# simonamtoft/downsampled-diffusion

Measured on AMD Instinct MI355X. Metric: images/sec (T=1000 sampling), 256x256 dDDPM-x3, higher is better.
Workload: dtype f32

## Files before the change

### downsampled-diffusion_amd/csrc/conv_igemm.hip

```cpp
#include <cstdlib>

#include "conv_common.h"

namespace ddk {

struct IgemmParams {
    const float* src0;
    const float* src1;
    const float* w;
    const float* bias;
    const float* resid;
    float* out;
    int c0, c1, cin;
    int B, H, W;
    int Hm, Wm;
    int Ho, Wo;
    int N, M;
    int in_stride, out_scale;
    int ntaps, nphase;
    int splits, kiters, kiters_per_split;
    long long slab_stride;
    int pre_mish, post_mish;
    float* mish_out;
    const float* dmish_src;
// ... 1161 lines not shown
        san::extent("conv resid", a.resid, pix_out * a.N * 4);
        san::extent("conv bias", a.bias, (long long)a.N * 4);
        san::extent("conv workspace", a.workspace, (long long)a.workspace_bytes);
        san::extent("conv mish_out", a.mish_out, pix_out * a.N * 4);
        san::extent("conv dmish_src", a.dmish_src, pix_out * a.N * 4);
        if (a.gn_partials && a.gn_groups > 0) san::extent("conv gn_partials", a.gn_partials, (pix_out / 128) * a.gn_groups * 8);
    }
#endif
    DDK_REQUIRE(aligned16(a.mish_out) && aligned16(a.dmish_src), "conv: mish_out / dmish_src alignment");
    DDK_REQUIRE(!(a.mish_out || a.dmish_src) || !(a.defer_reduce || a.gn_partials || fuse || ln),
                "conv: mish_out / dmish_src go with a plain conv (no deferred reduce, GroupNorm partials or LayerNorm folding)");
    const bool act_epilogue = a.mish_out || a.dmish_src;
    if (a.weight_wino && !a.pre_mish && !act_epilogue && conv_wino_ok(a.kind, a.H, a.W, a.c0 + a.c1, a.N)) {
        DDK_REQUIRE(aligned16(a.weight_wino), "conv: weight_wino alignment");
        DDK_TRY(ensure_device_init());
        const int ws = conv_wino_splits(a.B, a.H, a.W, a.c0 + a.c1, a.N);
        const long long slab = (long long)a.B * a.H * a.W * a.N;
        if (ws > 1) {
            const size_t need = (size_t)(fuse ? ws - 1 : ws) * slab * sizeof(float);
            if (!a.workspace || a.workspace_bytes < need) {
                set_error("conv(wino): split-K workspace too small (%zu < %zu)", a.workspace_bytes, need);
                return DDK_ERR_WORKSPACE;
            }
            DDK_REQUIRE(aligned16(a.workspace), "conv: workspace alignment");
        }
        DDK_REQUIRE((long long)a.B * a.H * a.W * (a.c0 > a.c1 ? a.c0 : a.c1) * 4 < (1LL << 31), "conv(wino): a source of 2 GiB or more");
        DDK_TRY(conv_wino_forward(a, ws, st, fuse));
        if (ws > 1 && !a.defer_reduce && !fuse) {
            const long long n4 = slab / 4;
            const int blocks = (int)(ceil_div(n4, 256) < 2048 ? ceil_div(n4, 256) : 2048);
            hipLaunchKernelGGL(splitk_reduce_kernel, dim3(blocks), dim3(256), 0, st, static_cast<const float*>(a.workspace), ws, slab, a.bias,
// ... 160 lines not shown
```

### downsampled-diffusion_amd/csrc/conv_wino.hip

```cpp
#include <atomic>
#include <cstdlib>
#include <type_traits>
#include <utility>

#include "cluster_sync.h"
#include "conv_common.h"
#include "pack_elems.h"

namespace ddk {

__device__ __attribute__((aligned(128))) float g_wino_zero[32];

struct WinoParams {
    const float* src0;
    const float* src1;
    const float* wu;
    const float* bias;
    const float* resid;
    float* out;
    int c0, c1, cin;
    int B, H, W, TH, TW;
    int N, tiles;
    int splits, chunks, chunks_per_split;
    long long slab_stride;
// ... 551 lines not shown
    DDK_HIP(hipFuncSetAttribute(reinterpret_cast<const void*>(&convT_wino_kernel<1>), hipFuncAttributeMaxDynamicSharedMemorySize,
                                (int)(WT_LDS_FL * sizeof(float))));
#endif
    DDK_HIP(hipFuncSetAttribute(reinterpret_cast<const void*>(&conv3x3_wino_kernel<0>), hipFuncAttributeMaxDynamicSharedMemorySize,
                                (int)(W_LDS_FLOATS * sizeof(float))));
    DDK_HIP(hipFuncSetAttribute(reinterpret_cast<const void*>(&conv3x3_wino_kernel<0, true>), hipFuncAttributeMaxDynamicSharedMemorySize,
                                (int)(W_LDS_FLOATS * sizeof(float))));
    DDK_HIP(hipFuncSetAttribute(reinterpret_cast<const void*>(&conv3x3_wino2_kernel<2, 0, false>), hipFuncAttributeMaxDynamicSharedMemorySize,
                                (int)(W2<2>::LDS_FL * sizeof(float))));
    DDK_HIP(hipFuncSetAttribute(reinterpret_cast<const void*>(&conv3x3_wino2_kernel<2, 0, true>), hipFuncAttributeMaxDynamicSharedMemorySize,
                                (int)(W2<2>::LDS_FL * sizeof(float))));
    DDK_HIP(hipFuncSetAttribute(reinterpret_cast<const void*>(&conv3x3_wino2_kernel<4, 0, false>), hipFuncAttributeMaxDynamicSharedMemorySize,
                                (int)(W2<4>::LDS_FL * sizeof(float))));
    DDK_HIP(hipFuncSetAttribute(reinterpret_cast<const void*>(&conv3x3_wino2_kernel<4, 0, true>), hipFuncAttributeMaxDynamicSharedMemorySize,
                                (int)(W2<4>::LDS_FL * sizeof(float))));
#ifdef DDK_TUNING
#define W2_DBG_ATTR(P_, D_) DDK_HIP(hipFuncSetAttribute(reinterpret_cast<const void*>(&conv3x3_wino2_kernel<P_, D_, false>), \
                                                hipFuncAttributeMaxDynamicSharedMemorySize, (int)(W2<P_>::LDS_FL * sizeof(float))))
    W2_DBG_ATTR(2, 1); W2_DBG_ATTR(2, 7); W2_DBG_ATTR(2, 9); W2_DBG_ATTR(2, 15); W2_DBG_ATTR(2, 17);
    W2_DBG_ATTR(4, 1); W2_DBG_ATTR(4, 7); W2_DBG_ATTR(4, 9); W2_DBG_ATTR(4, 15); W2_DBG_ATTR(4, 17);
#undef W2_DBG_ATTR
    DDK_HIP(hipFuncSetAttribute(reinterpret_cast<const void*>(&conv3x3_wino_kernel<1>), hipFuncAttributeMaxDynamicSharedMemorySize, (int)(W_LDS_FLOATS * sizeof(float))));
    DDK_HIP(hipFuncSetAttribute(reinterpret_cast<const void*>(&conv3x3_wino_kernel<2>), hipFuncAttributeMaxDynamicSharedMemorySize, (int)(W_LDS_FLOATS * sizeof(float))));
    DDK_HIP(hipFuncSetAttribute(reinterpret_cast<const void*>(&conv3x3_wino_kernel<3>), hipFuncAttributeMaxDynamicSharedMemorySize, (int)(W_LDS_FLOATS * sizeof(float))));
    DDK_HIP(hipFuncSetAttribute(reinterpret_cast<const void*>(&conv3x3_wino_kernel<4>), hipFuncAttributeMaxDynamicSharedMemorySize, (int)(W_LDS_FLOATS * sizeof(float))));
#endif
    return DDK_OK;
}

int conv_wino_cluster_np(int B, int H, int W, int cin, int N, int groups) {
// ... 12 lines not shown
int conv_wino_cluster_split_np(int B, int H, int W, int cin, int N, int groups, int* splits_out) {
    if (!conv_wino_ok(DDK_CONV3X3_S1, H, W, cin, N)) return 0;
    const int splits = conv_wino_splits(B, H, W, cin, N);
    if (splits_out) *splits_out = splits;
    if (splits <= 1 || splits > 4) return 0;
    const int np = wino_stats_shape_parts(B, H, W, cin, N, groups);
    if (np <= 0 || np > 8) return 0;
    const int variant = wino_variant(B, H, W, N);
    if (variant != WINO_V_D) return 0;
    const int nt_w = wino_nt(variant);
    if (N / groups > 32 || nt_w % (N / groups) || nt_w / (N / groups) > 8) return 0;
    const long long mt = (long long)B * np, nt = N / nt_w;
    if (mt * nt * splits > 256) return 0;
    return np;
}
size_t conv_wino_cluster_pair_words(int B, int H, int W, int N) {
    return (size_t)ceil_div((long long)B * (H / 2) * (W / 2), WBT) * (size_t)(N / WBN) * 16;
}
size_t conv_wino_cluster_ws_floats(int B, int H, int W, int N) {
    const long long mt = (long long)B * (H / 2) * (W / 2) / WBT, nt = N / WBN;
    return (size_t)(mt * nt * 32 + (long long)B * nt * 16);
}

bool conv_wino_cluster_device_ok() {
    static std::atomic<int> cached[64];
    int dev = 0;
    if (hipGetDevice(&dev) != hipSuccess || dev < 0 || dev >= 64) return false;
    int v = cached[dev].load(std::memory_order_relaxed);
    if (v == 0) {
        int cus = 0, xccs = 0;
        bool ok = hipDeviceGetAttribute(&cus, hipDeviceAttributeMultiprocessorCount, dev) == hipSuccess && cus == 256;
        ok = ok && hipDeviceGetAttribute(&xccs, hipDeviceAttributeNumberOfXccs, dev) == hipSuccess && xccs == 8;
        ok = ok && !getenv("HSA_CU_MASK") && !getenv("ROC_GLOBAL_CU_MASK");
        (void)hipGetLastError();
        v = ok ? 1 : 2;
        cached[dev].store(v, std::memory_order_relaxed);
    }
    return v == 1;
}

bool conv_wino_variant_new(int B, int H, int W, int N) { return wino_variant(B, H, W, N) != WINO_V_OLD; }

int conv_wino_forward(const ddk_conv_args& a, int splits, hipStream_t st, const WinoGnFuse* fuse) {
    WinoParams p{};
    if (fuse) {
        const int np = splits == 1 ? conv_wino_cluster_np(a.B, a.H, a.W, a.c0 + a.c1, a.N, fuse->groups)
                                   : conv_wino_cluster_split_np(a.B, a.H, a.W, a.c0 + a.c1, a.N, fuse->groups, nullptr);
        DDK_REQUIRE(np > 0 && !a.post_mish && !a.gn_partials, "conv(wino): shape not eligible for the in-launch GroupNorm");
        if (splits > 1) {
            DDK_REQUIRE(fuse->pairs && a.workspace && aligned16(a.workspace) && !fuse->res_x,
                        "conv(wino, cluster): a split shape needs pair counters and the slab workspace");
            p.cl_slab = static_cast<float*>(a.workspace);
            p.cl_pair = fuse->pairs;
        }
        DDK_REQUIRE(fuse->gamma && fuse->beta && fuse->records && fuse->counters && aligned16(fuse->gamma) && aligned16(fuse->beta) &&
                        aligned16(fuse->temb) && fuse->temb_stride % 4 == 0 && aligned16(fuse->records) && aligned16(fuse->counters),
                    "conv(wino): in-launch GroupNorm arguments");
        p.gn_gamma = fuse->gamma; p.gn_beta = fuse->beta; p.gn_temb = fuse->temb; p.gn_temb_rows = fuse->temb_rows;
        p.gn_temb_stride = fuse->temb_stride; p.gn_eps = fuse->eps;
        p.cl_rec = fuse->records; p.cl_cnt = fuse->counters; p.cl_fail = fuse->fail; p.cl_np = np;
        if (fuse->res_x) {
            DDK_REQUIRE(fuse->res_w && fuse->res_cin > 0 && fuse->res_cin <= 8 && fuse->res_ld >= fuse->res_cin && !a.resid,
// ... 13 lines not shown
        p.cpg = a.N / a.gn_groups;
    }
    p.src0 = a.src0; p.src1 = a.src1; p.wu = a.weight_wino; p.bias = a.bias; p.resid = a.resid; p.out = a.out;
    p.c0 = a.c0; p.c1 = a.c1; p.cin = a.c0 + a.c1;
    p.B = a.B; p.H = a.H; p.W = a.W; p.TH = a.H / 2; p.TW = a.W / 2;
    p.N = a.N; p.tiles = a.B * p.TH * p.TW;
    p.chunks = p.cin / 32;
    p.chunks_per_split = (int)ceil_div(p.chunks, splits);
    p.splits = (int)ceil_div(p.chunks, p.chunks_per_split);
    p.slab_stride = (long long)a.B * a.H * a.W * a.N;
    p.post_mish = a.post_mish;
    p.dTW = make_fastdiv_u((unsigned)p.TW);
    p.dTH = make_fastdiv_u((unsigned)p.TH);
    if (p.splits > 1 && !fuse) p.out = static_cast<float*>(a.workspace);
    const int variant = wino_variant(a.B, a.H, a.W, a.N);
    if (variant != WINO_V_OLD) {
        dim3 grid2((unsigned)ceil_div(p.tiles, WBT), (unsigned)(a.N / wino_nt(variant)), (unsigned)p.splits);
        const bool f = variant == WINO_V_F;
        const size_t lds = (size_t)(f ? W2<2>::LDS_FL : W2<4>::LDS_FL) * sizeof(float);
#ifdef DDK_TUNING
        if (getenv("DDK_WINO_STAMPS")) {
            const int v = getenv("DDK_WINO_DEBUG") ? atoi(getenv("DDK_WINO_DEBUG")) : 1;
#define W2_DBG_LAUNCH(D_)                                                                                              \
    if (v == D_) {                                                                                                     \
        if (f) hipLaunchKernelGGL((conv3x3_wino2_kernel<2, D_, false>), grid2, dim3(768), lds, st, p);                 \
        else hipLaunchKernelGGL((conv3x3_wino2_kernel<4, D_, false>), grid2, dim3(768), lds, st, p);                   \
        return check_launch("conv3x3_wino2_kernel<dbg>");                                                              \
    }
            W2_DBG_LAUNCH(7) W2_DBG_LAUNCH(9) W2_DBG_LAUNCH(15) W2_DBG_LAUNCH(17)
#undef W2_DBG_LAUNCH
// ... 145 lines not shown
}

extern "C" int ddk_conv3x3_gn_mish_cluster(const float* src0, int c0, const float* src1, int c1, const float* weight_wino, const float* bias,
                                           const float* gamma, const float* beta, const float* temb, int temb_stride, const float* addend,
                                           float* out, int B, int H, int W, int N, int groups, float eps, void* workspace,
                                           size_t workspace_bytes, ddk_stream_t s) {
    using namespace ddk;
    DDK_REQUIRE(src0 && weight_wino && gamma && beta && out && workspace, "conv3x3_gn_mish_cluster: null pointer");
    DDK_REQUIRE(conv_wino_cluster_device_ok() && ddk_conv3x3_gn_mish_cluster_ok(B, H, W, c0 + c1, N, groups) > 0,
                "conv3x3_gn_mish_cluster: shape or device not eligible (ddk_conv3x3_gn_mish_cluster_ok)");
    const size_t plain_bytes = ddk_conv3x3_gn_mish_cluster_workspace_bytes(B, H, W, N);
    const size_t split_bytes = ddk_conv3x3_gn_mish_cluster_split_workspace_bytes(B, H, W, c0 + c1, N, groups);
    DDK_REQUIRE(workspace_bytes >= (split_bytes ? split_bytes : plain_bytes) && aligned16(workspace), "conv3x3_gn_mish_cluster: workspace");
    float* ws = static_cast<float*>(workspace);
    DDK_HIP(hipMemsetAsync(ws, 0, ((size_t)B * 8 * 16 + 16) * sizeof(float), as_stream(s)));
    float* pairs = ws + plain_bytes / sizeof(float);
    if (split_bytes) DDK_HIP(hipMemsetAsync(pairs, 0, conv_wino_cluster_pair_words(B, H, W, N) * sizeof(float), as_stream(s)));
    ddk_conv_args a{};
    a.kind = DDK_CONV3X3_S1;
    a.src0 = src0; a.src1 = src1; a.c0 = c0; a.c1 = c1;
    a.weight = weight_wino;
    a.weight_wino = weight_wino;
    a.bias = bias;
    a.resid = addend;
    a.out = out;
    a.B = B; a.H = H; a.W = W; a.N = N;
    const ClWords w = cl_words(ws, B);
    WinoGnFuse f{gamma, beta, temb, nullptr, temb_stride, eps, groups, ws + (size_t)B * 8 * 16 + 16, w.counters, w.fail};
    if (split_bytes) {
        f.pairs = reinterpret_cast<unsigned*>(pairs);
        a.workspace = pairs + conv_wino_cluster_pair_words(B, H, W, N);
        a.workspace_bytes = split_bytes - plain_bytes - conv_wino_cluster_pair_words(B, H, W, N) * sizeof(float);
    }
    return conv_forward(a, as_stream(s), nullptr, &f);
}
```

### downsampled-diffusion_amd/csrc/conv_wino2_kernel.inc

```

template <int... I, class F>
__device__ __forceinline__ void static_for_impl(std::integer_sequence<int, I...>, F&& f) { (f(std::integral_constant<int, I>{}), ...); }
template <int N, class F>
__device__ __forceinline__ void static_for(F&& f) { static_for_impl(std::make_integer_sequence<int, N>{}, f); }

#ifndef DDK_WINO2_LP_F
#define DDK_WINO2_LP_F 8
#endif
#ifndef DDK_WINO2_LP_D
#define DDK_WINO2_LP_D 4
#endif
template <int P>
struct W2 {
    static constexpr int NT = 256 / P;
    static constexpr int NB = NT / 32;
    static constexpr int SPC = 16 / P;
    static constexpr int SPR = 4 / P;
    static constexpr int V_FL = P * WBT * 32;
    static constexpr int U_FL = P * NT * 32;
    static constexpr int STAGE = V_FL + U_FL;
    static constexpr int PPI = NT / 8;
    static constexpr int TP = NT + 4;
    static constexpr int T_FL = 4 * 2 * WBT * TP;
    static constexpr int LDS_FL = (3 * STAGE > T_FL + 320) ? 3 * STAGE : T_FL + 320;
    static constexpr int QUADS = NT / 4;
    static constexpr int ITEMS = 2 * WBT * QUADS / 512;
    static constexpr int LPL = P == 2 ? DDK_WINO2_LP_F : DDK_WINO2_LP_D;
    static constexpr int LPM = (32 - 4 * LPL) / 8;
    static_assert(4 * LPL + 8 * LPM == 32 && LPL % 2 == 0 && LPM % 2 == 0, "piece split: (8,0), (4,2) or (0,4)");
};
#ifndef DDK_WINO2_STAGGER
#define DDK_WINO2_STAGGER 1
#endif
constexpr bool W2_STAGGER = DDK_WINO2_STAGGER != 0;

__device__ unsigned long long g_wino_timeline[12 * 8 * 2];

template <int P, int DBG, bool CL>
__global__ __launch_bounds__(768) void conv3x3_wino2_kernel(const WinoParams p) {
    using G = W2<P>;
    constexpr int NT = G::NT, SPC = G::SPC, SPR = G::SPR, STAGE = G::STAGE, V_FL = G::V_FL;
    extern __shared__ __attribute__((aligned(16))) float smem[];
    unsigned long long r_entry = 0;
    if (DBG) r_entry = __builtin_amdgcn_s_memrealtime();
    const int tid = threadIdx.x, lane = tid & 63;
    const int wid = __builtin_amdgcn_readfirstlane(tid >> 6);
    int tile_m, tile_n, split;
    {
        const int nwg = gridDim.x * gridDim.y * gridDim.z;
        const int bid = blockIdx.x + gridDim.x * (blockIdx.y + gridDim.y * blockIdx.z);
        const int q = nwg >> 3, r = nwg & 7, xcd = bid & 7, idx = bid >> 3;
        const int logical = (xcd < r ? xcd * (q + 1) : r * (q + 1) + (xcd - r) * q) + idx;
        tile_n = logical % gridDim.y;
        const int rest = logical / gridDim.y;
        tile_m = rest % gridDim.x;
// ... 154 lines not shown
                unsigned long long tlA = 0;
                const bool tl = (DBG & 16) && blockIdx.x + blockIdx.y + blockIdx.z == 0 && S >= 8 && S < 16;
                if (tl) asm volatile("s_memtime %0\n\ts_waitcnt lgkmcnt(0)" : "=s"(tlA)::"memory");
                __builtin_amdgcn_s_barrier();
                if (tl) {
                    unsigned long long tlB;
                    asm volatile("s_memtime %0\n\ts_waitcnt lgkmcnt(0)" : "=s"(tlB)::"memory");
                    if (lane == 0) { g_wino_timeline[(wid * 8 + (S - 8)) * 2] = tlA; g_wino_timeline[(wid * 8 + (S - 8)) * 2 + 1] = tlB; }
                }
                b0 = b0 == 2 ? 0 : b0 + 1;
            });
        }
        return;
    }

    const int pp = wid % P, nb = wid / P;
    f32x16 acc[SPC];
#pragma unroll
    for (int i = 0; i < SPC; ++i)
#pragma unroll
        for (int r = 0; r < 16; ++r) acc[i][r] = 0.f;
    {
        const int fsw = ((lane & 31) >> 1) & 7, fh = lane >> 5;
        int foff[4];
#pragma unroll
        for (int q = 0; q < 4; ++q) foff[q] = (lane & 31) * 32 + (((2 * q + fh) ^ fsw) << 2);
        const int a_img = pp * (WBT * 32), b_img = V_FL + (pp * NT + nb * 32) * 32;
        if (G::LPM > 0 && !(DBG & 4)) {
            issue_u(0, 0, 4 * G::LPL + wid * G::LPM, std::integral_constant<int, G::LPM>{});
            issue_u(1, 1, 4 * G::LPL + wid * G::LPM, std::integral_constant<int, G::LPM>{});
            wait_vmcnt<G::LPM>();
// ... 66 lines not shown
                    if (more && !(DBG & 4)) wait_vmcnt<G::LPM>(); else wait_vmcnt<0>();
                    unsigned long long tA = 0, tB = 0;
                    if (DBG) { asm volatile("s_memtime %0\n\ts_waitcnt lgkmcnt(0)" : "=s"(tA)::"memory"); }
                    __builtin_amdgcn_s_barrier();
                    if (DBG) { asm volatile("s_memtime %0\n\ts_waitcnt lgkmcnt(0)" : "=s"(tB)::"memory"); c_wait += tB - tA; if (c_mma == 0) c_mma = tA; }
                    if ((DBG & 16) && blockIdx.x + blockIdx.y + blockIdx.z == 0 && S >= 8 && S < 16 && lane == 0) {
                        g_wino_timeline[(wid * 8 + (S - 8)) * 2] = tA;
                        g_wino_timeline[(wid * 8 + (S - 8)) * 2 + 1] = tB;
                    }
                    buf = nbuf;
                    ++S;
                });
            }
            if (STG) mma4(acc[SPC - 1], a[0], b[0]);
        };
        if (W2_STAGGER && wid >= 4) mloop(std::true_type{}); else mloop(std::false_type{});
        if (DBG && lane == 0 && wid == 0) {
            const int wg = (blockIdx.x + gridDim.x * (blockIdx.y + gridDim.y * blockIdx.z)) & 1023;
            unsigned long long tE;
            asm volatile("s_memtime %0\n\ts_waitcnt lgkmcnt(0)" : "=s"(tE)::"memory");
            g_wino_stamps[wg * 8 + 0] = r_entry;
            g_wino_stamps[wg * 8 + 1] = r_loop0;
            g_wino_stamps[wg * 8 + 2] = __builtin_amdgcn_s_memrealtime();
            g_wino_stamps[wg * 8 + 3] = c_wait;
            g_wino_stamps[wg * 8 + 4] = tE - c_mma;
            g_wino_stamps[wg * 8 + 5] = (unsigned long long)n_stages;
        }
    }
    {
        constexpr int TP = G::TP;
#pragma unroll
        for (int r = 0; r < 16; ++r) {
            const int row = (r & 3) + 8 * (r >> 2) + 4 * (lane >> 5);
            const int col = nb * 32 + (lane & 31);
            if constexpr (P == 4) {
                float* Ts = smem + pp * (2 * WBT * TP);
                const float m0 = acc[0][r], m1 = acc[1][r], m2 = acc[2][r], m3 = acc[3][r];
                Ts[row * TP + col] = (m0 + m1) + m2;
                Ts[(WBT + row) * TP + col] = (m1 - m2) - m3;
            } else {
                const float l0 = acc[0][r], l1 = acc[2][r], l2 = acc[4][r], l3 = acc[6][r];
                const float h0 = acc[1][r], h1 = acc[3][r], h2 = acc[5][r], h3 = acc[7][r];
                const float tl0 = (l0 + l1) + l2, tl1 = (l1 - l2) - l3;
                const float th0 = (h0 + h1) + h2, th1 = (h1 - h2) - h3;
                float* B0 = smem + (pp * 2 + 0) * (2 * WBT * TP);
                float* B1 = smem + (pp * 2 + 1) * (2 * WBT * TP);
                if (pp == 0) {
                    B0[row * TP + col] = tl0 + th0;          B0[(WBT + row) * TP + col] = tl1 + th1;
                    B1[row * TP + col] = -th0;               B1[(WBT + row) * TP + col] = -th1;
                } else {
                    B0[row * TP + col] = tl0;                B0[(WBT + row) * TP + col] = tl1;
                    B1[row * TP + col] = tl0 - th0;          B1[(WBT + row) * TP + col] = tl1 - th1;
                }
            }
        }
    }
    __syncthreads();

    constexpr int TP = G::TP, QUADS = G::QUADS, ITEMS = G::ITEMS;
    constexpr bool CLS = CL && P == 4;
    const bool partner = CLS && split > 0;
    const bool direct = p.splits == 1 || (CLS && !partner);
    float* outp = p.splits == 1 ? p.out : CLS ? p.cl_slab + (long long)(split - 1) * p.slab_stride : p.out + (long long)split * p.slab_stride;
    float4 keep[ITEMS][2];
    long long oo[ITEMS];
    int opix[ITEMS];
    const int cq = tid & (QUADS - 1);
    const int gn = n0 + cq * 4;
#pragma unroll
    for (int it = 0; it < ITEMS; ++it) {
        const int item = tid + it * 512;
        const int t = item / (2 * QUADS), a = (item / QUADS) & 1;
        const int g = t0 + t;
        keep[it][0] = keep[it][1] = make_float4(0.f, 0.f, 0.f, 0.f);
        oo[it] = -1;
        opix[it] = 0;
        if (g >= p.tiles || gn >= p.N) continue;
        const float* tp = smem + (a * WBT + t) * TP + cq * 4;
        const float4 q0 = *reinterpret_cast<const float4*>(tp);
        const float4 q1 = *reinterpret_cast<const float4*>(tp + 1 * (2 * WBT * TP));
        const float4 q2 = *reinterpret_cast<const float4*>(tp + 2 * (2 * WBT * TP));
        const float4 q3 = *reinterpret_cast<const float4*>(tp + 3 * (2 * WBT * TP));
        float4 y0, y1;
        if constexpr (P == 4) {
            y0 = f4add(f4add(q0, q1), q2);
            y1 = f4sub(f4sub(q1, q2), q3);
        } else {
            y0 = f4add(q0, q2);
            y1 = f4add(q1, q3);
        }
        const unsigned tmp = fdiv_u((unsigned)g, p.dTW);
        const int tx = g - (int)tmp * p.TW;
        const unsigned bq = fdiv_u(tmp, p.dTH);
        const int ty = (int)tmp - (int)bq * p.TH;
        const long long o0 = ((((long long)bq * p.H + 2 * ty + a) * p.W) + 2 * tx) * p.N + gn;
        oo[it] = o0;
        opix[it] = ((int)bq * p.H + 2 * ty + a) * p.W + 2 * tx;
        if (direct) {
            if (p.bias) {
// ... 8 lines not shown
            if (p.post_mish) {
                y0 = make_float4(mish_f(y0.x), mish_f(y0.y), mish_f(y0.z), mish_f(y0.w));
                y1 = make_float4(mish_f(y1.x), mish_f(y1.y), mish_f(y1.z), mish_f(y1.w));
            }
        }
        if (!CL) {
            *reinterpret_cast<float4*>(outp + o0) = y0;
            *reinterpret_cast<float4*>(outp + o0 + p.N) = y1;
        } else if (CLS && partner) {
            st_sc1_f4(outp + o0, y0);
            st_sc1_f4(outp + o0 + p.N, y1);
        }
        keep[it][0] = y0;
        keep[it][1] = y1;
    }
    if (CLS && p.splits > 1) {
        unsigned* pair = p.cl_pair + ((long long)tile_m * gridDim.y + tile_n) * 16;
        if (partner) {
            asm volatile("s_waitcnt vmcnt(0)" ::: "memory");
            __syncthreads();
            if (tid == 0) __hip_atomic_fetch_add(pair, 1u, __ATOMIC_RELAXED, __HIP_MEMORY_SCOPE_AGENT);
            return;
        }
        int* pair_gave_up = reinterpret_cast<int*>(smem + G::T_FL + 258);
        if (tid == 0) {
            *pair_gave_up = 0;
            const unsigned want = (unsigned)p.splits - 1u;
            if (cl_wait_ge<2>(pair, want, p.cl_fail)) *pair_gave_up = 1;
            __hip_atomic_store(pair, 0u, __ATOMIC_RELAXED, __HIP_MEMORY_SCOPE_AGENT);
        }
        __syncthreads();
// ... 155 lines not shown
```

### downsampled-diffusion_amd/csrc/ddk_internal.h

```cpp
#pragma once
#include <hip/hip_runtime.h>

#include <cstdarg>
#include <cstdint>
#include <cstdio>

#include "ddk.h"

#ifdef DDK_HOST_SANITIZE
#include "host_sanitize.h"
#endif

namespace ddk {

void set_error(const char* fmt, ...);

inline int fail_arg(const char* what) {
    set_error("bad argument: %s", what);
    return DDK_ERR_ARG;
}

inline int check_launch(const char* what) {
    hipError_t e = hipGetLastError();
    if (e != hipSuccess) {
// ... 93 lines not shown
    const float* c2;
    float eps;
};
struct WinoGnFuse {
    const float* gamma;
    const float* beta;
    const float* temb;
    const long long* temb_rows;
    int temb_stride;
    float eps;
    int groups;
    float* records;
    unsigned* counters;
    unsigned* fail;
    unsigned* pairs = nullptr;
    const float* res_x = nullptr;
    const float* res_w = nullptr;
    const float* res_b = nullptr;
    int res_cin = 0, res_ld = 0;
};
bool conv_ln_fold_ok(int B, int H, int W, int cin, int N);
int conv_forward(const ddk_conv_args& a, hipStream_t st, const ConvLnFold* ln = nullptr, const WinoGnFuse* fuse = nullptr);
int conv_splits(int kind, int B, int H, int W, int cin, int N);
bool conv_wino_ok(int kind, int H, int W, int cin, int N);
int conv_wino_splits(int B, int H, int W, int cin, int N);
int conv_wino_forward(const ddk_conv_args& a, int splits, hipStream_t st, const WinoGnFuse* fuse = nullptr);
int conv_wino_cluster_np(int B, int H, int W, int cin, int N, int groups);
int conv_wino_cluster_split_np(int B, int H, int W, int cin, int N, int groups, int* splits_out);
size_t conv_wino_cluster_pair_words(int B, int H, int W, int N);
bool conv_wino_variant_new(int B, int H, int W, int N);
bool conv_wino_cluster_device_ok();
size_t conv_wino_cluster_ws_floats(int B, int H, int W, int N);
unsigned conv_wino_cluster_timeouts();
unsigned conv_first_cluster_timeouts();
unsigned level_chain_cluster_timeouts();
struct ClWords { unsigned* counters; unsigned* fail; };
inline ClWords cl_words(float* cl, int B) { return {reinterpret_cast<unsigned*>(cl), reinterpret_cast<unsigned*>(cl + (size_t)B * 8 * 16)}; }
int cluster_fail_check(unsigned* word, hipStream_t st, const char* who, const char* tail);
bool convT_wino_ok(int H, int W, int cin, int N);
int convT_wino_splits(int B, int H, int W, int cin, int N);
int convT_wino_forward(const ddk_conv_args& a, int splits, hipStream_t st);
int conv_wino_init_device();
int conv_wino_stats_parts(int B, int H, int W, int cin, int N, int groups);
bool conv_first_ok(int cin, int N, int H, int W, int groups);
// ... 114 lines not shown
```

### downsampled-diffusion_amd/csrc/unet_plan.hip

```cpp
#include <algorithm>
#include <mutex>
#include <string>
#include <vector>

#include "ddk_internal.h"
#include "level_chain.h"

namespace ddk {

constexpr int HEADS = 4;
constexpr int HIDDEN = HEADS * 32;
constexpr int GROUPS = 8;
constexpr float GN_EPS = 1e-5f, LN_EPS = 1e-5f;

static inline int pad32(int c) { return (c + 31) / 32 * 32; }

enum PackKind { PK_COPY = 0, PK_CONV = 1, PK_CONVT = 2, PK_LINEAR_T = 3, PK_WINO = 4, PK_LOCAL = 5, PK_WLOCAL = 6, PK_FIRST = 7, PK_CONVT_WINO = 8,
                PK_ROWS = 9 , PK_LOCAL1 = 10 ,
                PK_CONVT_LOCAL = 11  };

struct Slot {
    std::string name;
    long long numel;
    int kind;
// ... 68 lines not shown
struct ddk_unet {
    std::mutex mu;
    std::vector<SamplerGraph> graphs;
    unsigned long long use_clock = 0;
    unsigned long long pack_epoch = 0;
    struct {
        const void* ws = nullptr;
        int t_start = -1, B = 0, H = 0, W = 0;
        unsigned long long pack_epoch = 0;
        std::vector<int64_t> map;
    } table;
    ddk_unet_config cfg;
    int cluster_gn = 1;
    int cluster_limit = 1 << 30;
    int cluster_np_max = 8;
    bool cluster_split = true;
    bool attn_kvctx = true;
    bool fold_down_reduce = false;
    bool first_gn = true;
    int level_chain = 9;
    int level_chain_max_batch = 32;
    int attn_fold_min_hw = 256;
    bool attn_fold = true;
    bool generic = false;
    std::vector<int> dimp;
    std::vector<Slot> slots;
    size_t packed_floats = 0;
    int L = 0;
    std::vector<int> dims;
    int time_dim = 0, temb_total = 0;
    size_t freqs = 0, w1t = 0, b1 = 0, w2t = 0, b2 = 0, temb_wt = 0, temb_bias = 0;
// ... 331 lines not shown
        std::lock_guard<std::mutex> lock(u->mu);
        u->cluster_limit = value;
        return DDK_OK;
    }
    if (option == 4) {
        std::lock_guard<std::mutex> lock(u->mu);
        if (!u->graphs.empty()) DDK_HIP(hipDeviceSynchronize());
        drop_graphs(u);
        u->cluster_np_max = value;
        return DDK_OK;
    }
    if (option == 11) {
        std::lock_guard<std::mutex> lock(u->mu);
        if (!u->graphs.empty()) DDK_HIP(hipDeviceSynchronize());
        drop_graphs(u);
        u->cluster_split = value != 0;
        return DDK_OK;
    }
    return fail_arg("unet_set_option: unknown option");
}
extern "C" unsigned ddk_debug_cluster_timeouts(void) {
    unsigned sum = 0;
    for (unsigned v : {ddk::conv_wino_cluster_timeouts(), ddk::conv_first_cluster_timeouts(), ddk::level_chain_cluster_timeouts()}) {
        if (v == ~0u) return ~0u;
        sum += v;
    }
    return sum;
}
extern "C" int ddk_unet_num_slots(const ddk_unet* u) { return u ? (int)u->slots.size() : 0; }
extern "C" const char* ddk_unet_slot_name(const ddk_unet* u, int slot) {
    return (u && slot >= 0 && slot < (int)u->slots.size()) ? u->slots[slot].name.c_str() : nullptr;
// ... 97 lines not shown
    return convT_wino_ok(H, W, cin, N) && convT_wino_splits(B, H, W, cin, N) <= 2;
}
static bool use_wino(const ConvW& cw, int H, int W, int cin, int N) {
    return cw.has_wu && conv_wino_ok(DDK_CONV3X3_S1, H, W, cin, N);
}
static int conv3_splits(const ConvW& cw, int B, int H, int W, int cin, int N) {
    return use_wino(cw, H, W, cin, N) ? conv_wino_splits(B, H, W, cin, N) : conv_splits(DDK_CONV3X3_S1, B, H, W, cin, N);
}
static size_t conv3_ws_floats(const ConvW& cw, int B, int H, int W, int cin, int N) {
    if (!use_wino(cw, H, W, cin, N)) return conv_workspace_bytes(DDK_CONV3X3_S1, B, H, W, cin, N) / 4;
    const int s = conv_wino_splits(B, H, W, cin, N);
    return s > 1 ? (size_t)s * B * H * W * N : 0;
}

constexpr size_t CL_PAIR_WORDS = 128 * 16;
static size_t cl_counter_floats(int B) { return (size_t)B * 8 * 16 + 16 + (size_t)B * 64 + CL_PAIR_WORDS; }
static size_t cl_chain_offset(int B) { return (size_t)B * 8 * 16 + 16; }
static size_t cl_pair_offset(int B) { return (size_t)B * 8 * 16 + 16 + (size_t)B * 64; }
constexpr int CHAIN_BUFS = 18;
constexpr int CHAIN8_BUFS = 5;

static void res_sizes(const ResW& r, int B, int H, int W, Layout& ly) {
    const size_t M = (size_t)B * H * W;
    upd(ly.act, M * r.co);
    upd(ly.splitk, conv3_ws_floats(r.c1, B, H, W, r.ci_pad, r.co));
    upd(ly.splitk, conv3_ws_floats(r.c2, B, H, W, r.co, r.co));
    if (r.has_res) upd(ly.splitk, conv_workspace_bytes(DDK_CONV1X1, B, H, W, r.ci_pad, r.co) / 4);
    upd(ly.gn_ws, groupnorm_workspace_bytes(B, H * W, r.co, GROUPS) / 4);
    upd(ly.gn_ws, (size_t)2 * GROUPS * (M / 128 + 1));
    upd(ly.cl, cl_counter_floats(B) + conv_wino_cluster_ws_floats(B, H, W, r.co));
    if (H * W % 128 == 0 && H * W / 128 <= 8) upd(ly.cl, cl_counter_floats(B) + conv_first_gn_ws_floats(B, H, W));
}

static void attn_sizes(const AttnW& a, int B, int H, int W, Layout& ly) {
    const size_t M = (size_t)B * H * W;
    upd(ly.act, M * a.c);
    upd(ly.qkv, M * 3 * HIDDEN);
    upd(ly.o, M * HIDDEN);
    upd(ly.ctx, (size_t)B * HEADS * 32 * 32);
    upd(ly.splitk, linattn_context_workspace_bytes(B, H * W, HEADS) / 4);
    if (attn_kvctx_ok(B, H * W, a.c, HEADS)) upd(ly.splitk, attn_kvctx_workspace_bytes(B, H * W) / 4);
    upd(ly.splitk, conv_workspace_bytes(DDK_CONV1X1, B, H, W, a.c, 3 * HIDDEN) / 4);
    upd(ly.splitk, conv_workspace_bytes(DDK_CONV1X1, B, H, W, HIDDEN, a.c) / 4);
}

// ... 140 lines not shown
    }
    const int cl_np = c.allow_cluster && cw.has_wu && conv_wino_cluster_device_ok() ? conv_wino_cluster_np(c.B, H, W, c0 + c1, N, GROUPS) : 0;
    if (cl_np > 0 && cl_np <= c.u.cluster_np_max && c.n_cluster++ < c.u.cluster_limit) {
        ddk_conv_args a{};
        a.kind = DDK_CONV3X3_S1;
        a.src0 = src0; a.src1 = src1; a.c0 = c0; a.c1 = c1;
        a.weight = c.P + cw.w;
        a.weight_wino = c.P + cw.wu;
        a.bias = cw.has_bias ? c.P + cw.b : nullptr;
        a.resid = addend;
        a.out = out;
        a.B = c.B; a.H = H; a.W = W; a.N = N;
        float* cl = c.W + c.ly.off_cl;
        const ClWords w = cl_words(cl, c.B);
        const WinoGnFuse f{c.P + n.g, c.P + n.b, temb, c.temb_rows, c.u.temb_total, GN_EPS, GROUPS, cl + cl_counter_floats(c.B), w.counters, w.fail};
        return conv_forward(a, c.st, nullptr, &f);
    }
    int cls_splits = 1;
    const int cls_np = c.allow_cluster && c.u.cluster_split && cw.has_wu && conv_wino_cluster_device_ok()
                           ? conv_wino_cluster_split_np(c.B, H, W, c0 + c1, N, GROUPS, &cls_splits) : 0;
    if (cls_np > 0 && cls_np <= c.u.cluster_np_max && (size_t)cls_splits * c.B * H * W * N <= c.ly.splitk &&
        conv_wino_cluster_pair_words(c.B, H, W, N) <= CL_PAIR_WORDS && c.n_cluster++ < c.u.cluster_limit) {
        ddk_conv_args a{};
        a.kind = DDK_CONV3X3_S1;
        a.src0 = src0; a.src1 = src1; a.c0 = c0; a.c1 = c1;
        a.weight = c.P + cw.w;
        a.weight_wino = c.P + cw.wu;
        a.bias = cw.has_bias ? c.P + cw.b : nullptr;
        a.resid = addend;
        a.out = out;
// ... 898 lines not shown
```

Before: 26.05.

## Add narrow-N Winograd cluster tile that splits K across waves in-block

Adds a narrow Winograd D-stage variant (32 output channels per block, 8 waves split as 4 phases by 2 K-halves) that runs at full K in one launch with in-block reduction of the two K halves, fused with in-launch GroupNorm. It is used for small-channel 3x3 convs (input channels up to 128) that previously needed a split-K cluster hand-off with pair words and a workspace memset. The cluster_split option becomes tri-state and defaults to the narrow path. The cost is a second wave-level reduction through LDS and fewer output channels per block, which means more blocks and more re-reads of the input tiles.

```diff
diff --git a/downsampled-diffusion_amd/csrc/conv_igemm.hip b/downsampled-diffusion_amd/csrc/conv_igemm.hip
--- a/downsampled-diffusion_amd/csrc/conv_igemm.hip
+++ b/downsampled-diffusion_amd/csrc/conv_igemm.hip
@@ -1199,7 +1199,7 @@
     if (a.weight_wino && !a.pre_mish && !act_epilogue && conv_wino_ok(a.kind, a.H, a.W, a.c0 + a.c1, a.N)) {
         DDK_REQUIRE(aligned16(a.weight_wino), "conv: weight_wino alignment");
         DDK_TRY(ensure_device_init());
-        const int ws = conv_wino_splits(a.B, a.H, a.W, a.c0 + a.c1, a.N);
+        const int ws = fuse && fuse->narrow ? 1 : conv_wino_splits(a.B, a.H, a.W, a.c0 + a.c1, a.N);
         const long long slab = (long long)a.B * a.H * a.W * a.N;
         if (ws > 1) {
             const size_t need = (size_t)(fuse ? ws - 1 : ws) * slab * sizeof(float);
diff --git a/downsampled-diffusion_amd/csrc/conv_wino.hip b/downsampled-diffusion_amd/csrc/conv_wino.hip
--- a/downsampled-diffusion_amd/csrc/conv_wino.hip
+++ b/downsampled-diffusion_amd/csrc/conv_wino.hip
@@ -589,6 +589,8 @@
                                 (int)(W2<4>::LDS_FL * sizeof(float))));
     DDK_HIP(hipFuncSetAttribute(reinterpret_cast<const void*>(&conv3x3_wino2_kernel<4, 0, true>), hipFuncAttributeMaxDynamicSharedMemorySize,
                                 (int)(W2<4>::LDS_FL * sizeof(float))));
+    DDK_HIP(hipFuncSetAttribute(reinterpret_cast<const void*>(&conv3x3_wino2_kernel<4, 0, true, true>), hipFuncAttributeMaxDynamicSharedMemorySize,
+                                (int)(W2<4, true>::LDS_FL * sizeof(float))));
 #ifdef DDK_TUNING
 #define W2_DBG_ATTR(P_, D_) DDK_HIP(hipFuncSetAttribute(reinterpret_cast<const void*>(&conv3x3_wino2_kernel<P_, D_, false>), \
                                                 hipFuncAttributeMaxDynamicSharedMemorySize, (int)(W2<P_>::LDS_FL * sizeof(float))))
@@ -631,6 +633,21 @@
     if (mt * nt * splits > 256) return 0;
     return np;
 }
+int conv_wino_cluster_narrow_np(int B, int H, int W, int cin, int N, int groups) {
+    if (!conv_wino_ok(DDK_CONV3X3_S1, H, W, cin, N) || conv_wino_splits(B, H, W, cin, N) <= 1) return 0;
+    if (wino_variant(B, H, W, N) != WINO_V_D || groups <= 0 || N % groups) return 0;
+    const int cpg = N / groups, tpi = (H / 2) * (W / 2);
+    if (cpg % 4 || 32 % cpg || tpi % WBT || tpi / WBT > 8) return 0;
+    const int np = tpi / WBT;
+    const long long mt = (long long)B * np, nt = N / 32;
+    if (nt > 8 || mt * nt > 256 || (mt * nt) % 8) return 0;
+    const long long run = mt * nt / 8, per_round = run < 32 ? run : 32;
+    if (run % (np * nt) || per_round % (np * nt)) return 0;
+    return np;
+}
+size_t conv_wino_cluster_narrow_ws_floats(int B, int H, int W, int N) {
+    return (size_t)ceil_div((long long)B * (H / 2) * (W / 2), WBT) * (size_t)(N / 32) * 32;
+}
 size_t conv_wino_cluster_pair_words(int B, int H, int W, int N) {
     return (size_t)ceil_div((long long)B * (H / 2) * (W / 2), WBT) * (size_t)(N / WBN) * 16;
 }
@@ -661,8 +678,10 @@
 int conv_wino_forward(const ddk_conv_args& a, int splits, hipStream_t st, const WinoGnFuse* fuse) {
     WinoParams p{};
     if (fuse) {
-        const int np = splits == 1 ? conv_wino_cluster_np(a.B, a.H, a.W, a.c0 + a.c1, a.N, fuse->groups)
-                                   : conv_wino_cluster_split_np(a.B, a.H, a.W, a.c0 + a.c1, a.N, fuse->groups, nullptr);
+        const int np = fuse->narrow ? conv_wino_cluster_narrow_np(a.B, a.H, a.W, a.c0 + a.c1, a.N, fuse->groups)
+                       : splits == 1 ? conv_wino_cluster_np(a.B, a.H, a.W, a.c0 + a.c1, a.N, fuse->groups)
+                                     : conv_wino_cluster_split_np(a.B, a.H, a.W, a.c0 + a.c1, a.N, fuse->groups, nullptr);
+        DDK_REQUIRE(!fuse->narrow || (splits == 1 && !fuse->pairs), "conv(wino, cluster): the narrow tile runs at full k");
         DDK_REQUIRE(np > 0 && !a.post_mish && !a.gn_partials, "conv(wino): shape not eligible for the in-launch GroupNorm");
         if (splits > 1) {
             DDK_REQUIRE(fuse->pairs && a.workspace && aligned16(a.workspace) && !fuse->res_x,
@@ -706,6 +725,12 @@
     p.dTH = make_fastdiv_u((unsigned)p.TH);
     if (p.splits > 1 && !fuse) p.out = static_cast<float*>(a.workspace);
     const int variant = wino_variant(a.B, a.H, a.W, a.N);
+    if (fuse && fuse->narrow) {
+        dim3 grid((unsigned)ceil_div(p.tiles, WBT), (unsigned)(a.N / 32), 1u);
+        const size_t lds = (size_t)W2<4, true>::LDS_FL * sizeof(float);
+        hipLaunchKernelGGL((conv3x3_wino2_kernel<4, 0, true, true>), grid, dim3(768), lds, st, p);
+        return check_launch("conv3x3_wino2_kernel<cluster, narrow>");
+    }
     if (variant != WINO_V_OLD) {
         dim3 grid2((unsigned)ceil_div(p.tiles, WBT), (unsigned)(a.N / wino_nt(variant)), (unsigned)p.splits);
         const bool f = variant == WINO_V_F;
@@ -881,8 +906,8 @@
     DDK_REQUIRE(workspace_bytes >= (split_bytes ? split_bytes : plain_bytes) && aligned16(workspace), "conv3x3_gn_mish_cluster: workspace");
     float* ws = static_cast<float*>(workspace);
     DDK_HIP(hipMemsetAsync(ws, 0, ((size_t)B * 8 * 16 + 16) * sizeof(float), as_stream(s)));
-    float* pairs = ws + plain_bytes / sizeof(float);
-    if (split_bytes) DDK_HIP(hipMemsetAsync(pairs, 0, conv_wino_cluster_pair_words(B, H, W, N) * sizeof(float), as_stream(s)));
+    const ClWords w = cl_words(ws, B);
+    WinoGnFuse f{gamma, beta, temb, nullptr, temb_stride, eps, groups, ws + (size_t)B * 8 * 16 + 16, w.counters, w.fail};
     ddk_conv_args a{};
     a.kind = DDK_CONV3X3_S1;
     a.src0 = src0; a.src1 = src1; a.c0 = c0; a.c1 = c1;
@@ -892,8 +917,13 @@
     a.resid = addend;
     a.out = out;
     a.B = B; a.H = H; a.W = W; a.N = N;
-    const ClWords w = cl_words(ws, B);
-    WinoGnFuse f{gamma, beta, temb, nullptr, temb_stride, eps, groups, ws + (size_t)B * 8 * 16 + 16, w.counters, w.fail};
+    if (split_bytes && conv_wino_cluster_narrow_np(B, H, W, c0 + c1, N, groups) > 0 &&
+        ((size_t)B * 8 * 16 + 16 + conv_wino_cluster_narrow_ws_floats(B, H, W, N)) * sizeof(float) <= workspace_bytes) {
+        f.narrow = true;
+        return conv_forward(a, as_stream(s), nullptr, &f);
+    }
+    float* pairs = ws + plain_bytes / sizeof(float);
+    if (split_bytes) DDK_HIP(hipMemsetAsync(pairs, 0, conv_wino_cluster_pair_words(B, H, W, N) * sizeof(float), as_stream(s)));
     if (split_bytes) {
         f.pairs = reinterpret_cast<unsigned*>(pairs);
         a.workspace = pairs + conv_wino_cluster_pair_words(B, H, W, N);
diff --git a/downsampled-diffusion_amd/csrc/conv_wino2_kernel.inc b/downsampled-diffusion_amd/csrc/conv_wino2_kernel.inc
--- a/downsampled-diffusion_amd/csrc/conv_wino2_kernel.inc
+++ b/downsampled-diffusion_amd/csrc/conv_wino2_kernel.inc
@@ -10,24 +10,31 @@
 #ifndef DDK_WINO2_LP_D
 #define DDK_WINO2_LP_D 4
 #endif
-template <int P>
+#ifndef DDK_WINO2_LP_N
+#define DDK_WINO2_LP_N 0
+#endif
+template <int P, bool NR = false>
 struct W2 {
-    static constexpr int NT = 256 / P;
+    static_assert(!NR || P == 4, "the narrow tile is a D stage");
+    static constexpr int NT = NR ? 32 : 256 / P;
     static constexpr int NB = NT / 32;
+    static constexpr int KH = NR ? 2 : 1;
+    static_assert(P * NB * KH == 8, "8 matrix waves");
     static constexpr int SPC = 16 / P;
     static constexpr int SPR = 4 / P;
     static constexpr int V_FL = P * WBT * 32;
     static constexpr int U_FL = P * NT * 32;
     static constexpr int STAGE = V_FL + U_FL;
     static constexpr int PPI = NT / 8;
+    static constexpr int PIECES = P * PPI;
     static constexpr int TP = NT + 4;
-    static constexpr int T_FL = 4 * 2 * WBT * TP;
+    static constexpr int T_FL = KH * 4 * 2 * WBT * TP;
     static constexpr int LDS_FL = (3 * STAGE > T_FL + 320) ? 3 * STAGE : T_FL + 320;
     static constexpr int QUADS = NT / 4;
     static constexpr int ITEMS = 2 * WBT * QUADS / 512;
-    static constexpr int LPL = P == 2 ? DDK_WINO2_LP_F : DDK_WINO2_LP_D;
-    static constexpr int LPM = (32 - 4 * LPL) / 8;
-    static_assert(4 * LPL + 8 * LPM == 32 && LPL % 2 == 0 && LPM % 2 == 0, "piece split: (8,0), (4,2) or (0,4)");
+    static constexpr int LPL = NR ? DDK_WINO2_LP_N : P == 2 ? DDK_WINO2_LP_F : DDK_WINO2_LP_D;
+    static constexpr int LPM = (PIECES - 4 * LPL) / 8;
+    static_assert(4 * LPL + 8 * LPM == PIECES && LPL % 2 == 0 && LPM % 2 == 0, "piece split: (8,0), (4,2) or (0,4); NR (4,0) or (0,2)");
 };
 #ifndef DDK_WINO2_STAGGER
 #define DDK_WINO2_STAGGER 1
@@ -36,9 +43,9 @@
 
 __device__ unsigned long long g_wino_timeline[12 * 8 * 2];
 
-template <int P, int DBG, bool CL>
+template <int P, int DBG, bool CL, bool NR = false>
 __global__ __launch_bounds__(768) void conv3x3_wino2_kernel(const WinoParams p) {
-    using G = W2<P>;
+    using G = W2<P, NR>;
     constexpr int NT = G::NT, SPC = G::SPC, SPR = G::SPR, STAGE = G::STAGE, V_FL = G::V_FL;
     extern __shared__ __attribute__((aligned(16))) float smem[];
     unsigned long long r_entry = 0;
@@ -223,7 +230,7 @@
         return;
     }
 
-    const int pp = wid % P, nb = wid / P;
+    const int pp = wid % P, nb = NR ? 0 : wid / P, kh = NR ? wid / P : 0;
     f32x16 acc[SPC];
 #pragma unroll
     for (int i = 0; i < SPC; ++i)
@@ -320,7 +327,47 @@
             }
             if (STG) mma4(acc[SPC - 1], a[0], b[0]);
         };
-        if (W2_STAGGER && wid >= 4) mloop(std::true_type{}); else mloop(std::false_type{});
+        auto mloop_nr = [&] {
+            const int fo0 = (lane & 31) * 32 + (((4 * kh + fh) ^ fsw) << 2);
+            const int fo1 = (lane & 31) * 32 + (((4 * kh + 2 + fh) ^ fsw) << 2);
+            float4 a0 = *reinterpret_cast<const float4*>(smem + a_img + fo0);
+            float4 a1 = *reinterpret_cast<const float4*>(smem + a_img + fo1);
+            int buf = 0, S = 0;
+            for (int c = 0; c < n_chunks; ++c) {
+                static_for<SPC>([&](auto sc) {
+                    constexpr int s = decltype(sc)::value;
+                    const float* Bs = smem + buf * STAGE + b_img;
+                    const int nbuf = buf == 2 ? 0 : buf + 1, pbuf = buf == 0 ? 2 : buf - 1;
+                    const bool more = S + 2 < n_stages;
+                    const float4 b0 = *reinterpret_cast<const float4*>(Bs + fo0);
+                    const float4 b1 = *reinterpret_cast<const float4*>(Bs + fo1);
+                    __builtin_amdgcn_sched_barrier(0);
+                    acc[s] = __builtin_amdgcn_mfma_f32_32x32x2f32(a0.x, b0.x, acc[s], 0, 0, 0);
+                    acc[s] = __builtin_amdgcn_mfma_f32_32x32x2f32(a0.y, b0.y, acc[s], 0, 0, 0);
+                    if (more && G::LPM > 0 && !(DBG & 4)) {
+                        __builtin_amdgcn_sched_barrier(0);
+                        issue_u(S + 2, pbuf, 4 * G::LPL + wid * G::LPM, std::integral_constant<int, G::LPM>{});
+                        __builtin_amdgcn_sched_barrier(0);
+                    }
+                    acc[s] = __builtin_amdgcn_mfma_f32_32x32x2f32(a0.z, b0.z, acc[s], 0, 0, 0);
+                    acc[s] = __builtin_amdgcn_mfma_f32_32x32x2f32(a0.w, b0.w, acc[s], 0, 0, 0);
+                    acc[s] = __builtin_amdgcn_mfma_f32_32x32x2f32(a1.x, b1.x, acc[s], 0, 0, 0);
+                    acc[s] = __builtin_amdgcn_mfma_f32_32x32x2f32(a1.y, b1.y, acc[s], 0, 0, 0);
+                    acc[s] = __builtin_amdgcn_mfma_f32_32x32x2f32(a1.z, b1.z, acc[s], 0, 0, 0);
+                    acc[s] = __builtin_amdgcn_mfma_f32_32x32x2f32(a1.w, b1.w, acc[s], 0, 0, 0);
+                    __builtin_amdgcn_sched_barrier(0);
+                    a0 = *reinterpret_cast<const float4*>(smem + nbuf * STAGE + a_img + fo0);
+                    a1 = *reinterpret_cast<const float4*>(smem + nbuf * STAGE + a_img + fo1);
+                    if (more && !(DBG & 4)) wait_vmcnt<G::LPM>(); else wait_vmcnt<0>();
+                    asm volatile("s_waitcnt lgkmcnt(0)" ::: "memory");
+                    __builtin_amdgcn_s_barrier();
+                    buf = nbuf;
+                    ++S;
+                });
+            }
+        };
+        if constexpr (NR) mloop_nr();
+        else if (W2_STAGGER && wid >= 4) mloop(std::true_type{}); else mloop(std::false_type{});
         if (DBG && lane == 0 && wid == 0) {
             const int wg = (blockIdx.x + gridDim.x * (blockIdx.y + gridDim.y * blockIdx.z)) & 1023;
             unsigned long long tE;
@@ -340,7 +387,7 @@
             const int row = (r & 3) + 8 * (r >> 2) + 4 * (lane >> 5);
             const int col = nb * 32 + (lane & 31);
             if constexpr (P == 4) {
-                float* Ts = smem + pp * (2 * WBT * TP);
+                float* Ts = smem + (kh * 4 + pp) * (2 * WBT * TP);
                 const float m0 = acc[0][r], m1 = acc[1][r], m2 = acc[2][r], m3 = acc[3][r];
                 Ts[row * TP + col] = (m0 + m1) + m2;
                 Ts[(WBT + row) * TP + col] = (m1 - m2) - m3;
@@ -364,7 +411,7 @@
     __syncthreads();
 
     constexpr int TP = G::TP, QUADS = G::QUADS, ITEMS = G::ITEMS;
-    constexpr bool CLS = CL && P == 4;
+    constexpr bool CLS = CL && P == 4 && !NR;
     const bool partner = CLS && split > 0;
     const bool direct = p.splits == 1 || (CLS && !partner);
     float* outp = p.splits == 1 ? p.out : CLS ? p.cl_slab + (long long)(split - 1) * p.slab_stride : p.out + (long long)split * p.slab_stride;
@@ -388,7 +435,14 @@
         const float4 q2 = *reinterpret_cast<const float4*>(tp + 2 * (2 * WBT * TP));
         const float4 q3 = *reinterpret_cast<const float4*>(tp + 3 * (2 * WBT * TP));
         float4 y0, y1;
-        if constexpr (P == 4) {
+        if constexpr (NR) {
+            const float4 r0 = *reinterpret_cast<const float4*>(tp + 4 * (2 * WBT * TP));
+            const float4 r1 = *reinterpret_cast<const float4*>(tp + 5 * (2 * WBT * TP));
+            const float4 r2 = *reinterpret_cast<const float4*>(tp + 6 * (2 * WBT * TP));
+            const float4 r3 = *reinterpret_cast<const float4*>(tp + 7 * (2 * WBT * TP));
+            y0 = f4add(f4add(f4add(q0, q1), q2), f4add(f4add(r0, r1), r2));
+            y1 = f4add(f4sub(f4sub(q1, q2), q3), f4sub(f4sub(r1, r2), r3));
+        } else if constexpr (P == 4) {
             y0 = f4add(f4add(q0, q1), q2);
             y1 = f4sub(f4sub(q1, q2), q3);
         } else {
@@ -427,7 +481,7 @@
         keep[it][0] = y0;
         keep[it][1] = y1;
     }
-    if (CLS && p.splits > 1) {
+    if constexpr (CLS) if (p.splits > 1) {
         unsigned* pair = p.cl_pair + ((long long)tile_m * gridDim.y + tile_n) * 16;
         if (partner) {
             asm volatile("s_waitcnt vmcnt(0)" ::: "memory");
diff --git a/downsampled-diffusion_amd/csrc/ddk_internal.h b/downsampled-diffusion_amd/csrc/ddk_internal.h
--- a/downsampled-diffusion_amd/csrc/ddk_internal.h
+++ b/downsampled-diffusion_amd/csrc/ddk_internal.h
@@ -131,6 +131,7 @@
     unsigned* counters;
     unsigned* fail;
     unsigned* pairs = nullptr;
+    bool narrow = false;
     const float* res_x = nullptr;
     const float* res_w = nullptr;
     const float* res_b = nullptr;
@@ -145,6 +146,8 @@
 int conv_wino_cluster_np(int B, int H, int W, int cin, int N, int groups);
 int conv_wino_cluster_split_np(int B, int H, int W, int cin, int N, int groups, int* splits_out);
 size_t conv_wino_cluster_pair_words(int B, int H, int W, int N);
+int conv_wino_cluster_narrow_np(int B, int H, int W, int cin, int N, int groups);
+size_t conv_wino_cluster_narrow_ws_floats(int B, int H, int W, int N);
 bool conv_wino_variant_new(int B, int H, int W, int N);
 bool conv_wino_cluster_device_ok();
 size_t conv_wino_cluster_ws_floats(int B, int H, int W, int N);
diff --git a/downsampled-diffusion_amd/csrc/unet_plan.hip b/downsampled-diffusion_amd/csrc/unet_plan.hip
--- a/downsampled-diffusion_amd/csrc/unet_plan.hip
+++ b/downsampled-diffusion_amd/csrc/unet_plan.hip
@@ -106,7 +106,7 @@
     int cluster_gn = 1;
     int cluster_limit = 1 << 30;
     int cluster_np_max = 8;
-    bool cluster_split = true;
+    int cluster_split = 2;
     bool attn_kvctx = true;
     bool fold_down_reduce = false;
     bool first_gn = true;
@@ -468,7 +468,8 @@
         std::lock_guard<std::mutex> lock(u->mu);
         if (!u->graphs.empty()) DDK_HIP(hipDeviceSynchronize());
         drop_graphs(u);
-        u->cluster_split = value != 0;
+        if (value < 0 || value > 2) return fail_arg("unet_set_option: option 11 takes 0 (off), 1 (k-split hand-off) or 2 (narrow tile)");
+        u->cluster_split = value;
         return DDK_OK;
     }
     return fail_arg("unet_set_option: unknown option");
@@ -596,6 +597,7 @@
 }
 
 constexpr size_t CL_PAIR_WORDS = 128 * 16;
+constexpr int NARROW_MAX_CHUNKS = 4;
 static size_t cl_counter_floats(int B) { return (size_t)B * 8 * 16 + 16 + (size_t)B * 64 + CL_PAIR_WORDS; }
 static size_t cl_chain_offset(int B) { return (size_t)B * 8 * 16 + 16; }
 static size_t cl_pair_offset(int B) { return (size_t)B * 8 * 16 + 16 + (size_t)B * 64; }
@@ -611,6 +613,7 @@
     upd(ly.gn_ws, groupnorm_workspace_bytes(B, H * W, r.co, GROUPS) / 4);
     upd(ly.gn_ws, (size_t)2 * GROUPS * (M / 128 + 1));
     upd(ly.cl, cl_counter_floats(B) + conv_wino_cluster_ws_floats(B, H, W, r.co));
+    upd(ly.cl, cl_counter_floats(B) + conv_wino_cluster_narrow_ws_floats(B, H, W, r.co));
     if (H * W % 128 == 0 && H * W / 128 <= 8) upd(ly.cl, cl_counter_floats(B) + conv_first_gn_ws_floats(B, H, W));
 }
 
@@ -781,6 +784,25 @@
         float* cl = c.W + c.ly.off_cl;
         const ClWords w = cl_words(cl, c.B);
         const WinoGnFuse f{c.P + n.g, c.P + n.b, temb, c.temb_rows, c.u.temb_total, GN_EPS, GROUPS, cl + cl_counter_floats(c.B), w.counters, w.fail};
+        return conv_forward(a, c.st, nullptr, &f);
+    }
+    const int nr_np = c.allow_cluster && c.u.cluster_split == 2 && c0 + c1 <= 32 * NARROW_MAX_CHUNKS && cw.has_wu && conv_wino_cluster_device_ok()
+                          ? conv_wino_cluster_narrow_np(c.B, H, W, c0 + c1, N, GROUPS) : 0;
+    if (nr_np > 0 && nr_np <= c.u.cluster_np_max && cl_counter_floats(c.B) + conv_wino_cluster_narrow_ws_floats(c.B, H, W, N) <= c.ly.cl &&
+        c.n_cluster++ < c.u.cluster_limit) {
+        ddk_conv_args a{};
+        a.kind = DDK_CONV3X3_S1;
+        a.src0 = src0; a.src1 = src1; a.c0 = c0; a.c1 = c1;
+        a.weight = c.P + cw.w;
+        a.weight_wino = c.P + cw.wu;
+        a.bias = cw.has_bias ? c.P + cw.b : nullptr;
+        a.resid = addend;
+        a.out = out;
+        a.B = c.B; a.H = H; a.W = W; a.N = N;
+        float* cl = c.W + c.ly.off_cl;
+        const ClWords w = cl_words(cl, c.B);
+        WinoGnFuse f{c.P + n.g, c.P + n.b, temb, c.temb_rows, c.u.temb_total, GN_EPS, GROUPS, cl + cl_counter_floats(c.B), w.counters, w.fail};
+        f.narrow = true;
         return conv_forward(a, c.st, nullptr, &f);
     }
     int cls_splits = 1;
```

Measured after the change: 26.21, median of 6. About the same (+0.6%).
